# lucadellalib/ts-asr

Measured on AMD Instinct MI355X. Metric: utterance-frames/sec (conformer-t_scratch training step, T=1000, B=32/GPU), higher is better.
Workload: dtype bf16; 1 GPU; BASELINE.json configs[1]: conformer-t_scratch 12L d256 (+6L speaker encoder), mel [32,1000,80] + enrollment mel [32,500,80] + tokens [32,120], injection cat, dropout 0.1, lens 1.0; global_batch=32, grad_accumulation_factor=1, parallelism=dp1, hip_graph=True

## Files before the change

include/tsasr_hip.h:

```cpp
#ifndef TSASR_HIP_H
#define TSASR_HIP_H
#include <stddef.h>
#include <stdint.h>

#ifdef __cplusplus
extern "C" {
#endif

#define TSASR_F32 0
#define TSASR_BF16 1

#define TSASR_E_INVALID (-1)
#define TSASR_E_LAUNCH (-2)
#define TSASR_E_WORKSPACE (-3)

const char *tsasr_last_error(void);
int tsasr_version(void);
int tsasr_device_ok(void);

int tsasr_joint_fwd(const void *enc, const void *dec, const float *W, const float *bias, float *logits,
                    int B, int T, int U1, int J, int V, int ldl, int io_dtype, float slope, void *stream);

int tsasr_joint_f32_fwd(const float *enc, const float *dec, const float *W, const float *bias, float *logits, int B, int T, int U1, int J, int V,
                        int ldl, float slope, void *stream);
// ... 77 lines not shown
                          float p, unsigned long long seed, const unsigned long long *seed_dev, const int32_t *valid_lens, int Trows,
                          int io_dtype, void *stream);
int tsasr_dropout_add_bwd(const void *dout, void *dx, float *dbias, long long M, int N, float alpha, float p,
                          unsigned long long seed, const unsigned long long *seed_dev, const int32_t *valid_lens, int Trows, int io_dtype,
                          void *workspace, size_t workspace_bytes, void *stream);
int tsasr_dropout_add2_fwd(const void *x, const float *bias, const void *res, void *out, long long M, int N, float alpha, float p,
                           unsigned long long seed, float p2, unsigned long long seed2, const unsigned long long *seed_dev,
                           const int32_t *valid_lens, int Trows, int io_dtype, void *stream);
int tsasr_dropout_add2_bwd(const void *dout, void *dx, void *dres, float *dbias, long long M, int N, float alpha, float p,
                           unsigned long long seed, float p2, unsigned long long seed2, const unsigned long long *seed_dev,
                           const int32_t *valid_lens, int Trows, int io_dtype, void *workspace, size_t workspace_bytes, void *stream);


int tsasr_convmod_fwd(const void *y2, const float *b2, const float *conv_w, const float *conv_b, const float *gamma,
                      const float *beta, void *z, void *c_save, float *mean, float *rstd, int B, int T, int D, int K, int causal,
                      float eps, float slope, int io_dtype, void *stream);
size_t tsasr_convmod_bwd_workspace_bytes(int B, int T, int D, int K);
int tsasr_convmod_bwd(const void *dz, const void *y2, const float *b2, const float *conv_w, const float *gamma, const float *beta,
                      const void *c_save, const float *mean, const float *rstd, void *dy2, float *dparams, int B, int T, int D,
                      int K, int causal, float slope, int io_dtype, void *workspace, size_t workspace_bytes, void *stream);


int tsasr_conv3x3s2_fwd(const void *x, const void *Wm, const float *b1, const void *W2, const float *b2, void *y1, void *y2, int B, int T, int F,
                        int Ci, int Co, int causal, void *stream);
size_t tsasr_conv3x3s2_wgrad_workspace_bytes(int B, int T, int F, int Ci);
int tsasr_conv3x3s2_wgrad(const void *dy1, const void *dy2, const void *x, float *dWm, float *dW2, int B, int T, int F, int Ci, int Co, int causal,
                          void *workspace, size_t workspace_bytes, void *stream);
int tsasr_conv3x3s2_wgrad_filters(const void *dy1, const void *dy2, const void *x, float *dW1, float *dW2, int B, int T, int F, int Ci, int Co, int causal,
                                  void *workspace, size_t workspace_bytes, void *stream);
size_t tsasr_conv3x3s2_dgrad_plan_bytes(int B, int T, int F, int causal);
int tsasr_conv3x3s2_dgrad_plan(int B, int T, int F, int causal, void *plan_host, size_t plan_bytes);
int tsasr_conv3x3s2_dgrad(const void *dy1, const void *dy2, const void *Wm, const void *W2, void *dx, int B, int T, int F, int Ci, int Co, int causal,
                          const void *plan_dev, size_t plan_bytes, void *stream);
int tsasr_frontend_out_len(int n);
int tsasr_frontend_c1_fwd(const void *x, const float *w1, const float *b1, const float *w2, const float *b2, void *y1, void *y2,
                          int B, int T, int F, int C, int causal, int io_dtype, void *stream);
size_t tsasr_frontend_c1_bwd_workspace_bytes(int C);
int tsasr_frontend_c1_bwd(const void *x, const void *dy1, const void *dy2, float *dparams, int B, int T, int F, int C, int causal,
                          int io_dtype, void *workspace, size_t workspace_bytes, void *stream);
int tsasr_frontend_im2col(const void *x, void *A, int B, int T, int F, int C, int causal, int io_dtype, void *stream);
int tsasr_frontend_col2im(const void *dA, const void *dR, void *dx, int B, int T, int F, int C, int causal, int io_dtype, void *stream);

int tsasr_frontend_block_supported(int Fo, int C);
int tsasr_frontend_block_fwd(const void *x, const void *y1, const void *y2, const float *w1, const float *b1, const float *w2,
                             const float *b2, const float *g1, const float *be1, const float *g2, const float *be2, void *out,
                             float *stats, int B, int T, int F, int C, int causal, float slope, float eps, float p_inner,
                             unsigned long long seed_inner, float p_outer, unsigned long long seed_outer,
                             const unsigned long long *seed_dev, int io_dtype, void *stream);
size_t tsasr_frontend_block_dparams(int Fo, int C, int with_conv);
size_t tsasr_frontend_block_bwd_workspace_bytes(int Fo, int C, int with_conv);
int tsasr_frontend_block_bwd(const void *x, const void *y1, const void *y2, const void *dout, const float *w1, const float *b1,
                             const float *w2, const float *b2, const float *g1, const float *be1, const float *g2,
                             const float *stats, void *dy1, void *dy2, float *dparams, int B, int T, int F, int C, int causal,
                             float slope, float p_inner, unsigned long long seed_inner, float p_outer,
                             unsigned long long seed_outer, const unsigned long long *seed_dev, int io_dtype, void *workspace,
                             size_t workspace_bytes, void *stream);


size_t tsasr_relpos_attn_lds_bytes(void);
int tsasr_relpos_attn_fwd(const void *qkv, const void *pk, const float *bias_u, const float *bias_v, const int32_t *key_lens,
                          void *out, float *lse, int B, int T, int H, int Dh, float scale, int causal, float pdrop,
                          unsigned long long seed, const unsigned long long *seed_dev, int io_dtype, void *stream);
size_t tsasr_relpos_attn_fwd_workspace_bytes(int B, int T, int H);
int tsasr_relpos_attn_fwd_ws(const void *qkv, const void *pk, const float *bias_u, const float *bias_v, const int32_t *key_lens,
                             void *out, float *lse, int B, int T, int H, int Dh, float scale, int causal, float pdrop,
                             unsigned long long seed, const unsigned long long *seed_dev, int io_dtype, void *workspace,
// ... 274 lines not shown
```

ts-asr_amd/_capi.py:

```python
import ctypes
import os

_HERE = os.path.dirname(os.path.abspath(__file__))
LIB_PATH = os.environ.get("TSASR_HIP_LIB") or os.path.join(_HERE, "lib", "libtsasr_hip.so")

F32, BF16 = 0, 1


class TsasrHipMissing(RuntimeError):
    pass


class TsasrHipError(RuntimeError):
    pass


_lib = None

c_void_p, c_int, c_float, c_size_t = ctypes.c_void_p, ctypes.c_int, ctypes.c_float, ctypes.c_size_t
c_double = ctypes.c_double
c_ll, c_ull = ctypes.c_longlong, ctypes.c_ulonglong

_PROTOS = {
    "tsasr_last_error": (ctypes.c_char_p, []),
# ... 23 lines not shown
    "tsasr_joint_wide_loss_error_word_offset": (ctypes.c_longlong, [c_int] * 5),
    "tsasr_joint_wide_loss_fwd": (c_int, [c_void_p] * 5 + [c_int] + [c_void_p] * 3 + [c_int] * 7 + [c_float, c_void_p, c_size_t, c_void_p]),
    "tsasr_joint_wide_loss_bwd": (c_int, [c_void_p] * 5 + [c_int] + [c_void_p] * 7 + [c_int] * 7 + [c_float, c_void_p, c_size_t, c_void_p]),
    "tsasr_joint_wide_align_workspace_bytes": (c_size_t, [c_int] * 5),
    "tsasr_joint_wide_align": (c_int, [c_void_p] * 5 + [c_int] + [c_void_p] * 3 + [c_int, c_void_p] + [c_int] * 7 + [c_float, c_void_p, c_size_t, c_void_p]),
    "tsasr_layernorm_fwd":(c_int, [c_void_p] * 6 + [c_ll, c_int, c_float, c_float, c_int, c_void_p]),
    "tsasr_layernorm_bwd_workspace_bytes": (c_size_t, [c_ll, c_int]),
    "tsasr_layernorm_bwd": (c_int, [c_void_p] * 9 + [c_ll, c_int, c_float, c_int, c_void_p, c_size_t, c_void_p]),
    "tsasr_layernorm_bwd_add": (c_int, [c_void_p] * 10 + [c_ll, c_int, c_float, c_int, c_void_p, c_size_t, c_void_p]),
    "tsasr_seed_advance": (c_int, [c_void_p, c_ull, c_void_p]),
    "tsasr_bias_act_dropout_fwd": (c_int, [c_void_p] * 3 + [c_ll, c_int, c_float, c_float, c_ull, c_void_p, c_int, c_void_p]),
    "tsasr_colpart_workspace_bytes": (c_size_t, [c_ll, c_int]),
    "tsasr_bias_act_dropout_bwd": (c_int, [c_void_p] * 4 + [c_ll, c_int, c_float, c_float, c_ull, c_void_p, c_int, c_void_p, c_size_t, c_void_p]),
    "tsasr_dropout_add_fwd": (c_int, [c_void_p] * 4 + [c_ll, c_int, c_float, c_float, c_ull, c_void_p, c_void_p, c_int, c_int, c_void_p]),
    "tsasr_dropout_add_bwd": (c_int, [c_void_p] * 3 + [c_ll, c_int, c_float, c_float, c_ull, c_void_p, c_void_p, c_int, c_int, c_void_p, c_size_t, c_void_p]),
    "tsasr_dropout_add2_fwd": (c_int, [c_void_p] * 4 + [c_ll, c_int, c_float, c_float, c_ull, c_float, c_ull, c_void_p, c_void_p, c_int, c_int, c_void_p]),
    "tsasr_dropout_add2_bwd": (c_int, [c_void_p] * 4 + [c_ll, c_int, c_float, c_float, c_ull, c_float, c_ull, c_void_p, c_void_p, c_int, c_int, c_void_p, c_size_t, c_void_p]),
    "tsasr_colsum_workspace_bytes": (c_size_t, [c_ll, c_int]),
    "tsasr_colsum": (c_int, [c_void_p, c_void_p, c_ll, c_int, c_int, c_int, c_void_p, c_size_t, c_void_p]),
    "tsasr_convmod_fwd": (c_int, [c_void_p] * 10 + [c_int] * 5 + [c_float, c_float, c_int, c_void_p]),
    "tsasr_convmod_bwd_workspace_bytes": (c_size_t, [c_int] * 4),
    "tsasr_convmod_bwd": (c_int, [c_void_p] * 11 + [c_int] * 5 + [c_float, c_int, c_void_p, c_size_t, c_void_p]),
    "tsasr_frontend_out_len": (c_int, [c_int]),
    "tsasr_frontend_c1_fwd": (c_int, [c_void_p] * 7 + [c_int] * 6 + [c_void_p]),
    "tsasr_frontend_c1_bwd_workspace_bytes": (c_size_t, [c_int]),
    "tsasr_frontend_c1_bwd": (c_int, [c_void_p] * 4 + [c_int] * 6 + [c_void_p, c_size_t, c_void_p]),
    "tsasr_conv3x3s2_fwd": (c_int, [c_void_p] * 7 + [c_int] * 6 + [c_void_p]),
    "tsasr_conv3x3s2_wgrad_workspace_bytes": (c_size_t, [c_int] * 4),
    "tsasr_conv3x3s2_wgrad": (c_int, [c_void_p] * 5 + [c_int] * 6 + [c_void_p, c_size_t, c_void_p]),
    "tsasr_conv3x3s2_wgrad_filters": (c_int, [c_void_p] * 5 + [c_int] * 6 + [c_void_p, c_size_t, c_void_p]),
    "tsasr_conv3x3s2_dgrad_plan_bytes": (c_size_t, [c_int] * 4),
    "tsasr_conv3x3s2_dgrad_plan": (c_int, [c_int] * 4 + [c_void_p, c_size_t]),
    "tsasr_conv3x3s2_dgrad": (c_int, [c_void_p] * 5 + [c_int] * 6 + [c_void_p, c_size_t, c_void_p]),
    "tsasr_frontend_im2col": (c_int, [c_void_p] * 2 + [c_int] * 6 + [c_void_p]),
    "tsasr_frontend_col2im": (c_int, [c_void_p] * 3 + [c_int] * 6 + [c_void_p]),
    "tsasr_frontend_block_supported": (c_int, [c_int, c_int]),
    "tsasr_frontend_block_fwd": (c_int, [c_void_p] * 13 + [c_int] * 5 + [c_float, c_float, c_float, c_ull, c_float, c_ull, c_void_p, c_int, c_void_p]),
    "tsasr_frontend_block_dparams": (c_size_t, [c_int] * 3),
    "tsasr_frontend_block_bwd_workspace_bytes": (c_size_t, [c_int] * 3),
    "tsasr_frontend_block_bwd": (c_int, [c_void_p] * 15 + [c_int] * 5 + [c_float, c_float, c_ull, c_float, c_ull, c_void_p, c_int, c_void_p, c_size_t, c_void_p]),
    "tsasr_relpos_attn_lds_bytes": (c_size_t, []),
    "tsasr_relpos_attn_fwd": (c_int, [c_void_p] * 7 + [c_int] * 4 + [c_float, c_int, c_float, c_ull, c_void_p, c_int, c_void_p]),
    "tsasr_relpos_attn_fwd_workspace_bytes": (c_size_t, [c_int] * 3),
    "tsasr_relpos_attn_fwd_ws": (c_int, [c_void_p] * 7 + [c_int] * 4 + [c_float, c_int, c_float, c_ull, c_void_p, c_int, c_void_p, c_size_t, c_void_p]),
    "tsasr_relpos_attn_bwd_workspace_bytes": (c_size_t, [c_int] * 3),
    "tsasr_relpos_attn_bwd": (c_int, [c_void_p] * 12 + [c_int] * 4 + [c_float, c_int, c_float, c_ull, c_void_p, c_int, c_void_p, c_size_t, c_void_p]),
    "tsasr_relpos_dpk_defer": (c_int, [c_int]),
    "tsasr_relpos_dpk_pending": (c_int, []),
    "tsasr_relpos_dpk_table_bytes": (c_size_t, [c_int]),
    "tsasr_relpos_dpk_flush": (c_int, [c_void_p, c_void_p, c_size_t, c_void_p]),
    "tsasr_relpos_dpk_discard": (None, []),
    "tsasr_relpos_attn_keepbits_bytes": (c_size_t, [c_int] * 3),
    "tsasr_relpos_attn_keepbits": (None, [c_void_p]),
    "tsasr_accumulate_many": (c_int, [c_void_p, c_int, c_void_p]),
    "tsasr_clip_adamw_workspace_bytes": (c_size_t, []),
    "tsasr_clip_adamw_step": (c_int, [c_void_p] * 8 + [c_ll] + [c_float] * 5 + [c_void_p, c_size_t, c_void_p]),
    "tsasr_gemm_set_plan": (None, [c_int, c_int]),
    "tsasr_gemm_set_ring": (None, [c_int]),
    "tsasr_gemm_set_lab_floor": (None, [c_int]),
    "tsasr_gemm_bf16_workspace_bytes": (c_size_t, [c_int] * 4),
    "tsasr_gemm_f32": (c_int, [c_void_p] * 3 + [c_int] * 3 + [c_ll] * 3 + [c_int] * 3 + [c_void_p]),
    "tsasr_gemm_bf16_nt_batched": (c_int, [c_void_p] * 3 + [c_int] * 3 + [c_ll] * 4 + [c_int, c_void_p]),
    "tsasr_gemm_bf16_fused_workspace_bytes": (c_size_t, [c_int] * 2),
    "tsasr_gemm_bf16_fused": (c_int, [c_void_p] * 3 + [c_int] * 3 + [c_ll] * 3 + [c_int] * 3 + [c_void_p, c_void_p, c_ll, c_float, c_float, c_ull, c_void_p, c_void_p, c_void_p, c_void_p, c_size_t, c_void_p]),
    "tsasr_gemm_bf16_fused_mask_ok": (c_int, [c_int] * 3),
    "tsasr_gemm_bf16": (c_int, [c_void_p] * 3 + [c_int] * 3 + [c_ll] * 3 + [c_int] * 4 + [c_void_p, c_size_t, c_void_p]),
# ... 177 lines not shown
```

ts-asr_amd/csrc/gemm.hip:

```cpp
#include <stdlib.h>
#include <string.h>

#include <algorithm>
#include <utility>
#include <vector>

#include "common.h"

#define GB_K 64

typedef __attribute__((address_space(3))) bf16x4 lds_bf16x4_t;

struct EpiArgs {
    int mode;
    const float *bias;
    const bf16_t *y;
    long long ldy;
    float slope, p;
    unsigned long long seed;
    const unsigned long long *seed_dev;
    float *colpart;
    const void *const *btab;
    long long c_batch;
};

template <int BM, int BN, bool AT, bool BT>
struct GemmSmem {
    static constexpr int A_LD = AT ? (BM + 32) : (GB_K + 8);
    static constexpr int B_LD = BT ? (BN + 32) : (GB_K + 8);
    static constexpr int A_ELEMS = AT ? GB_K * A_LD : BM * A_LD;
    static constexpr int B_ELEMS = BT ? GB_K * B_LD : BN * B_LD;
    static constexpr int STAGE = A_ELEMS + B_ELEMS;
    static constexpr size_t PIPE_BYTES = (size_t)2 * STAGE * sizeof(bf16_t);
    static constexpr size_t EPI_BYTES = (size_t)BM * (BN + 4) * sizeof(float);
    static constexpr size_t BYTES = PIPE_BYTES > EPI_BYTES ? PIPE_BYTES : EPI_BYTES;
};
// ... 1045 lines not shown
        const char *as = smem + (kt % RING_STAGES) * SLOT, *bs = as + TA::BYTES;
        bf16x8 af[2][NS], bfr[NS];
#pragma unroll
        for (int s = 0; s < NS; ++s) {
#pragma unroll
            for (int i = 0; i < 2; ++i) af[i][s] = TA::frag_at(as, a_off[i][s]);
            bfr[s] = TB::frag_at(bs, b_off[s]);
        }
#pragma unroll
        for (int s = 0; s < NS; ++s)
#pragma unroll
            for (int i = 0; i < 2; ++i) acc[i] = __builtin_amdgcn_mfma_f32_32x32x16_bf16(af[i][s], bfr[s], acc[i], 0, 0, 0);
    }
    asm volatile("s_waitcnt lgkmcnt(0)" ::: "memory");
    __builtin_amdgcn_s_barrier();
    constexpr int LDT = 64 + 8;
    bf16_t *tl = reinterpret_cast<bf16_t *>(smem);
    const int r = lane & 31, hh = lane >> 5;
#pragma unroll
    for (int i = 0; i < 2; ++i)
#pragma unroll
        for (int gq = 0; gq < 16; ++gq) tl[(wm * 64 + 32 * i + (gq & 3) + 8 * (gq >> 2) + 4 * hh) * LDT + wn * 32 + r] = (bf16_t)acc[i][gq];
    __syncthreads();
    for (int e = threadIdx.x; e < 128 * 8; e += 256) {
        const int rr = e >> 3, cc = (e & 7) * 8;
        const int row = r0 + rr;
        if (row >= c.rows) continue;
        const unsigned q = (unsigned)row / (unsigned)c.nf, fi_i = (unsigned)row - q * (unsigned)c.nf, b = q / (unsigned)c.nt, ti_i = q - b * (unsigned)c.nt;
        const long long pix = ((long long)b * g.T + c.t0 + c.tstep * (int)ti_i) * g.F + c.f0 + c.fstep * (int)fi_i;
        *reinterpret_cast<uint4 *>(dx + pix * g.Ci + n0 + cc) = *reinterpret_cast<const uint4 *>(tl + rr * LDT + cc);
    }
}

struct ConvAxisClass { int i0, step, n, ostep, ns, k[4], c[4]; };
static int conv_src_index_host(int o, int k, int n, int mode) {
    if (mode == 1) { const int i = 2 * o + k - 2; return i < 0 ? -1 : i; }
    int i = 2 * o + k - 1;
    if (mode == 0) { if (i < 0) i = -i; if (i >= n) i = 2 * (n - 1) - i; return i; }
    return (i < 0 || i >= n) ? -1 : i;
}
static bool conv_dgrad_axis(int n, int No, int mode, std::vector<ConvAxisClass> &out) {
    std::vector<std::vector<std::pair<int, int>>> L(n);
    for (int o = 0; o < No; ++o)
        for (int k = 0; k < 3; ++k) {
            const int i = conv_src_index_host(o, k, n, mode);
            if (i >= 0) L[i].push_back({k, o});
        }
    const int off = mode == 1 ? 2 : 1;
    std::vector<char> regular(n);
    for (int i = 0; i < n; ++i) {
        std::vector<std::pair<int, int>> e;
        for (int k = 0; k < 3; ++k)
            if (((i - k + off) & 1) == 0) {
                const int o = (i - k + off) / 2;
                if (i - k + off >= 0 && o < No) e.push_back({k, o});
            }
        std::sort(e.begin(), e.end());
        std::sort(L[i].begin(), L[i].end());
        regular[i] = e == L[i];
    }
    for (int i = 0; i < n; ++i) {
        if (regular[i]) {
            if (i >= 2 && regular[i - 2]) continue;
            ConvAxisClass a{};
            a.i0 = i; a.step = 2; a.ostep = 1; a.n = 0;
            for (int j = i; j < n && regular[j]; j += 2) ++a.n;
// ... 207 lines not shown
        p.splits = cdiv(K, p.kchunk);
        return p;
    }
    const long long t0 = (long long)cdiv(M, 128) * cdiv(N, 128), t1 = (long long)cdiv(M, 128) * cdiv(N, 64),
                    t2 = (long long)cdiv(M, 64) * cdiv(N, 64);
    static const int thr0 = 512, thr1 = 192;
    p.tile = t0 >= thr0 ? 0 : (t1 >= thr1 ? 1 : 2);
    const long long tiles = p.tile == 0 ? t0 : (p.tile == 1 ? t1 : t2);
    p.splits = 1;
    static const int min_k = 384;
    if (out_f32 && tiles < 256 && K >= min_k) {
        static const int target = 768;
        int s = (int)((target + tiles - 1) / tiles);
        const int max_s = std::max(1, K / (min_k >= 1024 ? 256 : 128));
        if (s > max_s) s = max_s;
        if (s > 32) s = 32;
        if (s < 1) s = 1;
        p.splits = s;
    }
    p.kchunk = cdiv(cdiv(K, p.splits), GB_K) * GB_K;
    p.splits = cdiv(K, p.kchunk);
    return p;
}

template <int OUT_MODE>
static void launch_tile(int tile, int tA, int tB, const void *A, const void *B, void *C, int M, int N, int K, long long lda, long long ldb,
                        long long ldc, int splits, int kchunk, long long slab_stride, hipStream_t st, const EpiArgs &ep = EpiArgs{}) {
    if (tile == 0) launch_t<128, 128, OUT_MODE>(tA, tB, A, B, C, M, N, K, lda, ldb, ldc, splits, kchunk, slab_stride, st, ep);
    else if (tile == 1) launch_t<128, 64, OUT_MODE>(tA, tB, A, B, C, M, N, K, lda, ldb, ldc, splits, kchunk, slab_stride, st, ep);
    else launch_t<64, 64, OUT_MODE>(tA, tB, A, B, C, M, N, K, lda, ldb, ldc, splits, kchunk, slab_stride, st, ep);
}

static int tile_bm(int tile) { return tile == 2 ? 64 : 128; }

extern "C" {

void tsasr_gemm_set_ring(int on) { g_use_ring = on; }
void tsasr_gemm_set_plan(int tile, int splits) { g_force_tile = tile; g_force_splits = splits; }
void tsasr_gemm_set_lab_floor(int floor_mode) { g_lab_floor = floor_mode; }

size_t tsasr_gemm_bf16_workspace_bytes(int M, int N, int K, int out_dtype) {
    const GemmPlan p = plan(M, N, K, out_dtype == TSASR_F32);
    return p.splits > 1 ? align_up((size_t)p.splits * M * N * sizeof(float), 256) : 0;
}

int tsasr_gemm_bf16(const void *A, const void *B, void *C, int M, int N, int K, long long lda, long long ldb, long long ldc,
                    int transA, int transB, int out_dtype, int accumulate, void *workspace, size_t workspace_bytes, void *stream) {
    TSASR_CHECK_ARG(A && B && C, "tsasr_gemm_bf16: null pointer");
    TSASR_CHECK_ARG(M > 0 && N > 0 && K > 0, "tsasr_gemm_bf16: empty problem (%d,%d,%d)", M, N, K);
    TSASR_CHECK_ARG(lda % 8 == 0 && ldb % 8 == 0 && (transA ? M : K) % 8 == 0 && (transB ? N : K) % 8 == 0,
                    "tsasr_gemm_bf16: rows must be multiples of 8 bf16 (M=%d N=%d K=%d lda=%lld ldb=%lld)", M, N, K, lda, ldb);
    TSASR_CHECK_ARG(out_dtype == TSASR_BF16 || out_dtype == TSASR_F32, "tsasr_gemm_bf16: bad out_dtype %d", out_dtype);
    TSASR_CHECK_ARG(!(accumulate && out_dtype != TSASR_F32), "tsasr_gemm_bf16: accumulate needs fp32 output");
    const GemmPlan p = plan(M, N, K, out_dtype == TSASR_F32);
    hipStream_t st = (hipStream_t)stream;
    static const bool log_small = false;
    if (log_small && (long long)cdiv(M, tile_bm(p.tile)) * cdiv(N, p.tile == 0 ? 128 : 64) * p.splits <= 16)
        fprintf(stderr, "[tsasr_gemm_bf16] few tiles: M=%d N=%d K=%d tA=%d tB=%d out=%d acc=%d tile=%d splits=%d\n", M, N, K, transA, transB, out_dtype, accumulate, p.tile, p.splits);
    if (p.splits > 1) {
        TSASR_CHECK_ARG(workspace && workspace_bytes >= tsasr_gemm_bf16_workspace_bytes(M, N, K, out_dtype), "tsasr_gemm_bf16: workspace too small");
        TSASR_CHECK_ARG(N % 4 == 0 && ldc % 4 == 0, "tsasr_gemm_bf16: split-K output needs N, ldc multiples of 4");
        const long long ss = (long long)M * N;
        launch_tile<1>(p.tile, transA, transB, A, B, workspace, M, N, K, lda, ldb, N, p.splits, p.kchunk, ss, st);
        if (accumulate == 2 && ldc == N && ss < (1ll << 31) && tsasr_reduce_deferring())
            tsasr_reduce_submit((const float *)workspace, (float *)C, ss, p.splits, (int)ss, 1, st);
        else
// ... 89 lines not shown
    const int s1 = conv_wgrad_splits(P, 9 * Ci), s2 = conv_wgrad_splits(P, Ci);
    float *slab2 = (float *)((char *)workspace + align_up((size_t)s1 * 128 * 9 * Ci * sizeof(float), 256));
    const int kc1 = (int)(((P + s1 - 1) / s1 + GB_K - 1) / GB_K * GB_K), kc2 = (int)(((P + s2 - 1) / s2 + GB_K - 1) / GB_K * GB_K);
    const int z1 = (int)((P + kc1 - 1) / kc1), z2 = (int)((P + kc2 - 1) / kc2);
    conv_s2_wgrad_kernel<<<(unsigned)((9 * Ci / 64) * 2 * z1), RING_THREADS, lds, st>>>((const bf16_t *)dy1, (const bf16_t *)x, slab1, g, P, 0, 9 * Ci, kc1, z1);
    conv_s2_wgrad_kernel<<<(unsigned)((Ci / 64) * 2 * z2), RING_THREADS, lds, st>>>((const bf16_t *)dy2, (const bf16_t *)x, slab2, g, P, (causal ? 7 : 4) * Ci, Ci, kc2, z2);
    if (filter_layout) conv_filter_reduce_kernel<<<(unsigned)cdiv(128 * 9 * Ci, 256), 256, 0, st>>>(slab1, dWm, Ci, z1, (long long)128 * 9 * Ci);
    else gemm_slab_reduce_kernel<<<(unsigned)cdiv(128 * 9 * Ci / 4, 256), 256, 0, st>>>(slab1, dWm, 128, 9 * Ci, 9 * Ci, z1, (long long)128 * 9 * Ci, 0);
    gemm_slab_reduce_kernel<<<(unsigned)cdiv(128 * Ci / 4, 256), 256, 0, st>>>(slab2, dW2, 128, Ci, Ci, z2, (long long)128 * Ci, 0);
    TSASR_CHECK_LAUNCH("tsasr_conv3x3s2_wgrad");
    return 0;
}

size_t tsasr_conv3x3s2_dgrad_plan_bytes(int B, int T, int F, int causal) {
    ConvDgradPlan pl;
    if (B <= 0 || T < 2 || F < 2 || !conv_dgrad_plan(B, T, F, causal, false, pl)) return 0;
    return (size_t)(CONV_DGRAD_HDR + 32 * pl.cls.size() + 2 * (size_t)pl.slots) * sizeof(int);
}
int tsasr_conv3x3s2_dgrad_plan(int B, int T, int F, int causal, void *plan_host, size_t plan_bytes) {
    TSASR_CHECK_ARG(plan_host && B > 0 && T >= 2 && F >= 2, "tsasr_conv3x3s2_dgrad_plan: bad argument");
    ConvDgradPlan pl;
    TSASR_CHECK_ARG(conv_dgrad_plan(B, T, F, causal, true, pl), "tsasr_conv3x3s2_dgrad_plan: unsupported shape (T=%d F=%d)", T, F);
    const size_t need = (size_t)(CONV_DGRAD_HDR + 32 * pl.cls.size() + 2 * (size_t)pl.slots) * sizeof(int);
    TSASR_CHECK_ARG(plan_bytes >= need, "tsasr_conv3x3s2_dgrad_plan: buffer too small");
    int *p = (int *)plan_host;
    memset(p, 0, need);
    p[0] = (int)pl.cls.size(); p[1] = pl.slots; p[2] = CONV_DGRAD_HDR; p[3] = CONV_DGRAD_HDR + 32 * (int)pl.cls.size();
    p[4] = B; p[5] = T; p[6] = F; p[7] = causal ? 1 : 0;
    static_assert(sizeof(ConvDgradClass) == 32 * sizeof(int), "class record = 32 ints");
    memcpy(p + p[2], pl.cls.data(), pl.cls.size() * sizeof(ConvDgradClass));
    for (int w = 0; w < pl.slots; ++w) { p[p[3] + 2 * w] = pl.tile_cls[w]; p[p[3] + 2 * w + 1] = pl.tile_idx[w]; }
    return 0;
}
int tsasr_conv3x3s2_dgrad(const void *dy1, const void *dy2, const void *Wm, const void *W2, void *dx, int B, int T, int F, int Ci, int Co, int causal,
                          const void *plan_dev, size_t plan_bytes, void *stream) {
    TSASR_CHECK_ARG(dy1 && dy2 && Wm && W2 && dx && plan_dev, "tsasr_conv3x3s2_dgrad: null pointer");
    TSASR_CHECK_ARG(B > 0 && T >= 2 && F >= 2 && Co == 128 && Ci % 64 == 0 && Ci >= 64 && Ci <= 128, "tsasr_conv3x3s2_dgrad: unsupported shape (Ci=%d Co=%d)", Ci, Co);
    ConvGeom g{B, T, F, (T - 1) / 2 + 1, (F - 1) / 2 + 1, Ci, causal ? 1 : 0, causal ? 2 : 0};
    TSASR_CHECK_ARG((long long)B * T * F < (1ll << 31), "tsasr_conv3x3s2_dgrad: more than 2^31 positions");
    ConvDgradPlan pl;
    TSASR_CHECK_ARG(conv_dgrad_plan(B, T, F, causal, false, pl), "tsasr_conv3x3s2_dgrad: unsupported shape (T=%d F=%d)", T, F);
    TSASR_CHECK_ARG(plan_bytes >= (size_t)(CONV_DGRAD_HDR + 32 * pl.cls.size() + 2 * (size_t)pl.slots) * sizeof(int), "tsasr_conv3x3s2_dgrad: plan of another shape");
    constexpr int lds = RING_STAGES * (RingTile<128, false>::BYTES + RingTile<64, true>::BYTES);
    (void)hipFuncSetAttribute((const void *)conv_s2_dgrad_kernel, hipFuncAttributeMaxDynamicSharedMemorySize, lds);
    conv_s2_dgrad_kernel<<<dim3((unsigned)pl.slots, (unsigned)(Ci / 64)), RING_THREADS, lds, (hipStream_t)stream>>>(
        (const bf16_t *)dy1, (const bf16_t *)dy2, (const bf16_t *)Wm, (const bf16_t *)W2, (bf16_t *)dx, g, (const int *)plan_dev);
    TSASR_CHECK_LAUNCH("tsasr_conv3x3s2_dgrad");
    return 0;
}

size_t tsasr_gemm_bf16_fused_workspace_bytes(int M, int N) { return align_up((size_t)cdiv(M, 64) * N * sizeof(float), 256); }

int tsasr_gemm_bf16_fused_mask_ok(int M, int N, int K) { return (g_force_tile < 0 && tsasr_gemm_big_bm(M, N, K)) ? 1 : 0; }

int tsasr_gemm_bf16_fused(const void *A, const void *B, void *C, int M, int N, int K, long long lda, long long ldb, long long ldc,
                          int transA, int transB, int epi_mode, const float *bias, const void *y, long long ldy, float slope, float p,
                          unsigned long long seed, const unsigned long long *seed_dev, float *dbias, void *mask, void *workspace,
                          size_t workspace_bytes, void *stream) {
    TSASR_CHECK_ARG(A && B && C, "tsasr_gemm_bf16_fused: null pointer");
    TSASR_CHECK_ARG(M > 0 && N > 0 && K > 0 && N % 8 == 0 && ldc % 8 == 0, "tsasr_gemm_bf16_fused: N and ldc must be multiples of 8");
    TSASR_CHECK_ARG(lda % 8 == 0 && ldb % 8 == 0 && (transA ? M : K) % 8 == 0 && (transB ? N : K) % 8 == 0, "tsasr_gemm_bf16_fused: rows must be multiples of 8 bf16");
    TSASR_CHECK_ARG(epi_mode == 1 || (epi_mode == 2 && y && ldy % 8 == 0), "tsasr_gemm_bf16_fused: bad epilogue mode %d", epi_mode);
    TSASR_CHECK_ARG(!mask || (!transA && !transB && tsasr_gemm_bf16_fused_mask_ok(M, N, K)), "tsasr_gemm_bf16_fused: no mask words for this shape (ask tsasr_gemm_bf16_fused_mask_ok)");
    TSASR_CHECK_ARG(p >= 0.f && p < 1.f, "tsasr_gemm_bf16_fused: bad dropout %f", p);
    TSASR_CHECK_ARG(!(mask && slope > 1.f), "tsasr_gemm_bf16_fused: mask words need a LeakyReLU slope in [0, 1] (or none), got %f", slope);
    TSASR_CHECK_ARG(!(epi_mode == 2 && dbias) || (workspace && workspace_bytes >= tsasr_gemm_bf16_fused_workspace_bytes(M, N)), "tsasr_gemm_bf16_fused: workspace too small");
    GemmPlan pl = plan(M, N, K, 0);
    hipStream_t st = (hipStream_t)stream;
    static const bool log_small = false;
    if (log_small && (long long)cdiv(M, tile_bm(pl.tile)) * cdiv(N, pl.tile == 0 ? 128 : 64) <= 16)
        fprintf(stderr, "[tsasr_gemm_bf16_fused] few tiles: M=%d N=%d K=%d tA=%d tB=%d mode=%d tile=%d\n", M, N, K, transA, transB, epi_mode, pl.tile);
    if (!transA && !transB && g_force_tile < 0) {
        const int bm = tsasr_gemm_big_bm(M, N, K);
        float *colpart = (epi_mode == 2 && dbias) ? (float *)workspace : nullptr;
        if (bm && tsasr_gemm_big_launch(A, B, C, M, N, K, lda, ldb, ldc, epi_mode, bias, y, ldy, slope, p, seed, seed_dev, colpart, mask, st) == 0) {
            if (colpart) tsasr_reduce_submit(colpart, dbias, N, cdiv(M, bm), N, 0, st);
            TSASR_CHECK_LAUNCH("tsasr_gemm_bf16_fused");
            return 0;
        }
    }
    EpiArgs ep{};
// ... 10 lines not shown
```

ts-asr_amd/ops.py:

```python
import math
import os

import torch
import torch.nn.functional as F

from . import _capi as C
from . import prof

STATUS = {
    "joint_logits": "HIP", "rnnt_loss": "HIP", "layer_norm": "HIP", "bias_act_dropout": "HIP", "dropout_add": "HIP",
    "convmod_core": "HIP",
    "frontend_c1": "HIP", "frontend_im2col/col2im": "HIP (fp32 / other channel counts)",
    "frontend block 1 (bf16)": "HIP (frontend_block.hip: convolutions and filter gradients on MFMA)",
    "frontend block 2 (bf16, C_out = 128)": "HIP implicit GEMMs (conv_s2_fwd / conv_s2_wgrad / conv_s2_dgrad)",
    "matmul(bf16)": "HIP (gemm_bf16: fwd, dgrad, wgrad-into-arena)", "matmul(fp32 parity mode)": "HIP (gemm_f32: fp32 matrix cores; fwd, dgrad, wgrad)", "lstm(bf16 training)": "HIP persistent whole-sequence kernels (per-step kernels for other H)", "lstm(decoding / fp32 parity)": "HIP (lstm_f32: exact fp32, optional initial state)",
    "attention(fp32 parity, cross_attention injection)": "HIP (attention_f32: exact fp32)", "joint(fp32 parity)": "HIP (joint_f32)",
    "joint(32 < V <= 1024: subword vocabularies)": "HIP (joint_wide.hip: vocabulary tiles inside the kernels; bf16-rounded h / W / dlogits with bf16 OR fp32 activations - "
                                                   "an exact-fp32 wide joint is not built: compute_dtype fp32 with V > 32 runs these kernels with fp32 storage)",
    "joint + loss without logits (joint_logits: lazy, 32 < V <= 1024)": "HIP (joint_wide.hip: joint_wide_lp / joint_wide_lazy_x / joint_wide_lazy_w; V <= 32 materialises)",
    "greedy search (V <= 1024, embedding <= 1024 columns)": "HIP (search.hip: greedy_decode_kernel for V <= 63 / E <= 64, greedy_decode_wide_kernel above)",
    "beam search / LM fusion with V > 63 or an embedding past 64 columns (V, E <= 1024, beam_size <= 64)":
        "HIP (search.hip: beam_search_wide_kernel, workgroup-wide log-softmax and top-k; offline, streams, timestamps and LM fusion)",
    "injection sum / prod": "HIP (inject)", "mix_sources": "HIP (dataio.hip)", "fbank": "HIP", "sentence_norm": "HIP", "fbank_frames": "HIP", "running_norm": "HIP (features_stream.hip)",
    "fbank_frames_slots": "HIP (features.hip: the fbank frame body over per-slot sample rings)", "audio_ring_append": "HIP (features_stream.hip)",
# ... 1567 lines not shown
        C.require_gpu(x)
        xc = x.contiguous()
        B, T, Fq = xc.shape
        Co = w1.shape[0]
        f = lambda t: _f32(t).contiguous()
        y1 = torch.empty(B, _out_len(T), _out_len(Fq), Co, dtype=xc.dtype, device=xc.device)
        y2 = torch.empty_like(y1)
        with prof.region("frontend_c1_fwd"):
            C.check(C.lib().tsasr_frontend_c1_fwd(C.ptr(xc), C.ptr(f(w1)), C.ptr(f(b1)), C.ptr(f(w2)), C.ptr(f(b2)), C.ptr(y1), C.ptr(y2),
                                                  B, T, Fq, Co, int(causal), C.io_dtype(xc), C.stream_ptr()), "tsasr_frontend_c1_fwd")
        ctx.save_for_backward(xc)
        ctx.cfg = (bool(causal), Co, (w1, b1, w2, b2))
        return y1, y2

    @staticmethod
    def backward(ctx, dy1, dy2):
        (xc,) = ctx.saved_tensors
        causal, Co, prm = ctx.cfg
        B, T, Fq = xc.shape
        dpar = torch.empty(Co * 12, dtype=torch.float32, device=xc.device)
        _keep(dpar)
        ws = _ws(C.lib().tsasr_frontend_c1_bwd_workspace_bytes(Co), xc.device)
        with prof.region("frontend_c1_bwd"):
            C.check(C.lib().tsasr_frontend_c1_bwd(C.ptr(xc), C.ptr(dy1.contiguous()), C.ptr(dy2.contiguous()), C.ptr(dpar), B, T, Fq, Co,
                                                  int(causal), C.io_dtype(xc), C.ptr(ws), ws.numel(), C.stream_ptr()), "tsasr_frontend_c1_bwd")
        return (None, _pgrad(prm[0], dpar[:Co * 9]), _pgrad(prm[1], dpar[Co * 9:Co * 10]), _pgrad(prm[2], dpar[Co * 10:Co * 11]),
                _pgrad(prm[3], dpar[Co * 11:]), None)


CONV_IMPLICIT = os.environ.get("TSASR_CONV_IMPLICIT", "1") != "0"


CONV_DGRAD_IMPLICIT = os.environ.get("TSASR_CONV_DGRAD", "1") != "0"
_CONV_DGRAD_PLANS = {}


def _conv_dgrad_plan(B, T, Fq, causal, device):
    key = (B, T, Fq, bool(causal), str(device))
    if key not in _CONV_DGRAD_PLANS:
        if torch.cuda.is_current_stream_capturing():
            raise RuntimeError("front-end data-gradient plan requested for a new shape during graph capture: run one eager step of this shape first")
        n = C.lib().tsasr_conv3x3s2_dgrad_plan_bytes(B, T, Fq, int(causal))
        if n == 0:
            _CONV_DGRAD_PLANS[key] = None
        else:
            host = torch.empty(n // 4, dtype=torch.int32)
            C.check(C.lib().tsasr_conv3x3s2_dgrad_plan(B, T, Fq, int(causal), host.data_ptr(), n), "tsasr_conv3x3s2_dgrad_plan")
            _CONV_DGRAD_PLANS[key] = host.to(device)
    return _CONV_DGRAD_PLANS[key]


def _pgrad_view(dwm, Co, Ci, dtype):
    return dwm.view(Co, 3, 3, Ci).permute(0, 3, 2, 1).to(dtype)


def _pgrad_view2(dw2f, shape, dtype):
    return dw2f.view(shape).to(dtype)


class _FrontendConvFn(torch.autograd.Function):

    @staticmethod
    def forward(ctx, x, w1, b1, w2, b2, causal):
        C.require_gpu(x)
        xc = x.contiguous()
        B, T, Fq, Ci = xc.shape
# ... 26 lines not shown
        elif xc.dtype == torch.float32 and _F32_HIP_GEMM:
            y1 = (gemm_f32(A, wm, P, Co, 9 * Ci, 9 * Ci, 9 * Ci, 0, 0) + b1.float()).view(B, To, Fo, Co)
            y2 = (gemm_f32(A[:, centre * Ci:], w2m, P, Co, Ci, 9 * Ci, Ci, 0, 0) + b2.float()).view(B, To, Fo, Co)
        else:
            lib_fallback("frontend conv block 2", f"{xc.dtype}, fp32 HIP GEMM off")
            Ac = A.view(P, 9, Ci)[:, centre, :]
            y1 = F.linear(A, wm, b1.to(xc.dtype)).view(B, To, Fo, Co)
            y2 = F.linear(Ac, w2m, b2.to(xc.dtype)).view(B, To, Fo, Co)
        ctx.implicit = False
        ctx.save_for_backward(A, wm, w2m)
        ctx.cfg = (bool(causal), (B, T, Fq, Ci), Co, centre, w1.dtype, b1.dtype, w2.dtype, b2.dtype, w2.shape, hip)
        ctx.biases = (b1, b2)
        return y1, y2

    @staticmethod
    def backward(ctx, dy1, dy2):
        A, wm, w2m = ctx.saved_tensors
        causal, (B, T, Fq, Ci), Co, centre, dw1t, db1t, dw2t, db2t, w2shape, hip = ctx.cfg
        P = B * _out_len(T) * _out_len(Fq)
        g1, g2 = dy1.reshape(P, Co).contiguous(), dy2.reshape(P, Co).contiguous()
        if ctx.implicit:
            xc = A
            dwm = torch.empty(Co, Ci, 3, 3, dtype=torch.float32, device=xc.device)
            dw2f = torch.empty(Co, Ci, dtype=torch.float32, device=xc.device)
            ws = _ws(C.lib().tsasr_conv3x3s2_wgrad_workspace_bytes(B, T, Fq, Ci), xc.device)
            with prof.region("conv3x3s2_wgrad", 2.0 * P * Co * 10 * Ci):
                C.check(C.lib().tsasr_conv3x3s2_wgrad_filters(C.ptr(g1), C.ptr(g2), C.ptr(xc), C.ptr(dwm), C.ptr(dw2f), B, T, Fq, Ci, Co, int(causal),
                                                              C.ptr(ws), ws.numel(), C.stream_ptr()), "tsasr_conv3x3s2_wgrad_filters")
            db1, db2 = _pgrad(ctx.biases[0], colsum(g1)), _pgrad(ctx.biases[1], colsum(g2))
            dx = torch.empty(B, T, Fq, Ci, dtype=xc.dtype, device=xc.device)
            plan = _conv_dgrad_plan(B, T, Fq, causal, xc.device) if CONV_DGRAD_IMPLICIT else None
            if plan is not None:
                with prof.region("conv3x3s2_dgrad", 2.0 * P * Co * 10 * Ci):
                    C.check(C.lib().tsasr_conv3x3s2_dgrad(C.ptr(g1), C.ptr(g2), C.ptr(wm), C.ptr(w2m), C.ptr(dx), B, T, Fq, Ci, Co, int(causal),
                                                          C.ptr(plan), plan.numel() * 4, C.stream_ptr()), "tsasr_conv3x3s2_dgrad")
            else:
                dA = gemm_bf16(g1, wm, P, 9 * Ci, Co, Co, 9 * Ci, 0, 1)
                dR = gemm_bf16(g2, w2m, P, Ci, Co, Co, Ci, 0, 1)
                with prof.region("frontend_col2im"):
                    C.check(C.lib().tsasr_frontend_col2im(C.ptr(dA), C.ptr(dR), C.ptr(dx), B, T, Fq, Ci, int(causal), C.io_dtype(xc), C.stream_ptr()),
                            "tsasr_frontend_col2im")
            return dx, _pgrad(ctx.weights[0], dwm.to(dw1t)), db1, _pgrad(ctx.weights[1], dw2f.to(dw2t)), db2, None
        if hip:
            dwm = gemm_bf16(g1, A, Co, 9 * Ci, P, Co, 9 * Ci, 1, 1, out_dtype=torch.float32)
            dw2 = gemm_bf16(g2, A[:, centre * Ci:], Co, Ci, P, Co, 9 * Ci, 1, 1, out_dtype=torch.float32).view(w2shape).to(dw2t)
            dA = gemm_bf16(g1, wm, P, 9 * Ci, Co, Co, 9 * Ci, 0, 1)
            dR = gemm_bf16(g2, w2m, P, Ci, Co, Co, Ci, 0, 1)
        elif A.dtype == torch.float32 and _F32_HIP_GEMM:
            dwm = gemm_f32(g1, A, Co, 9 * Ci, P, Co, 9 * Ci, 1, 1)
            dw2 = gemm_f32(g2, A[:, centre * Ci:], Co, Ci, P, Co, 9 * Ci, 1, 1).view(w2shape).to(dw2t)
            dA = gemm_f32(g1, wm, P, 9 * Ci, Co, Co, 9 * Ci, 0, 1)
            dR = gemm_f32(g2, w2m, P, Ci, Co, Co, Ci, 0, 1)
        else:
            dwm = g1.t() @ A
            dw2 = (g2.t() @ A.view(P, 9, Ci)[:, centre, :]).view(w2shape).to(dw2t)
            dA = g1 @ wm
            dR = g2 @ w2m
        dw1 = dwm.view(Co, 3, 3, Ci).permute(0, 3, 2, 1).to(dw1t)
        if hip:
            db1, db2 = _pgrad(ctx.biases[0], colsum(g1)), _pgrad(ctx.biases[1], colsum(g2))
        else:
            db1, db2 = g1.sum(0, dtype=torch.float32).to(db1t), g2.sum(0, dtype=torch.float32).to(db2t)
        dx = torch.empty(B, T, Fq, Ci, dtype=A.dtype, device=A.device)
        with prof.region("frontend_col2im"):
            C.check(C.lib().tsasr_frontend_col2im(C.ptr(dA), C.ptr(dR), C.ptr(dx), B, T, Fq, Ci, int(causal), C.io_dtype(A), C.stream_ptr()),
                    "tsasr_frontend_col2im")
        return dx, dw1, db1, dw2, db2, None

# ... 766 lines not shown
```

Measured before the change: 3.270 million frames/s.

## Add persistent warp-specialized conv3x3s2 dgrad kernel with producer DMA waves

Adds a persistent version of the stride-2 conv data-gradient kernel. Four producer waves stream A/B tiles into a 3-stage LDS ring via global_load_lds, while eight consumer waves run MFMA and write dx through an LDS staging buffer. The grid is capped at the CU count and walks the plan's tile list, and BN=128 lets each tile cover both Ci halves. The host-side plan rebuild on every call is also replaced by a small cached shape table. This is meant to cut launch/tail overhead and hide load latency in the front-end backward, at the cost of a single WG per CU and more complex barrier-count coupling between the two wave groups.

```diff
diff --git a/include/tsasr_hip.h b/include/tsasr_hip.h
--- a/include/tsasr_hip.h
+++ b/include/tsasr_hip.h
@@ -133,6 +133,9 @@
 int tsasr_conv3x3s2_dgrad_plan(int B, int T, int F, int causal, void *plan_host, size_t plan_bytes);
 int tsasr_conv3x3s2_dgrad(const void *dy1, const void *dy2, const void *Wm, const void *W2, void *dx, int B, int T, int F, int Ci, int Co, int causal,
                           const void *plan_dev, size_t plan_bytes, void *stream);
+int tsasr_conv3x3s2_dgrad_impl(const void *dy1, const void *dy2, const void *Wm, const void *W2, void *dx, int B, int T, int F, int Ci, int Co,
+                               int causal, const void *plan_dev, size_t plan_bytes, int impl, void *stream);
+void tsasr_conv3x3s2_dgrad_next_wgs(int wgs);
 int tsasr_frontend_out_len(int n);
 int tsasr_frontend_c1_fwd(const void *x, const float *w1, const float *b1, const float *w2, const float *b2, void *y1, void *y2,
                           int B, int T, int F, int C, int causal, int io_dtype, void *stream);
diff --git a/ts-asr_amd/_capi.py b/ts-asr_amd/_capi.py
--- a/ts-asr_amd/_capi.py
+++ b/ts-asr_amd/_capi.py
@@ -79,6 +79,8 @@
     "tsasr_conv3x3s2_dgrad_plan_bytes": (c_size_t, [c_int] * 4),
     "tsasr_conv3x3s2_dgrad_plan": (c_int, [c_int] * 4 + [c_void_p, c_size_t]),
     "tsasr_conv3x3s2_dgrad": (c_int, [c_void_p] * 5 + [c_int] * 6 + [c_void_p, c_size_t, c_void_p]),
+    "tsasr_conv3x3s2_dgrad_impl": (c_int, [c_void_p] * 5 + [c_int] * 6 + [c_void_p, c_size_t, c_int, c_void_p]),
+    "tsasr_conv3x3s2_dgrad_next_wgs": (None, [c_int]),
     "tsasr_frontend_im2col": (c_int, [c_void_p] * 2 + [c_int] * 6 + [c_void_p]),
     "tsasr_frontend_col2im": (c_int, [c_void_p] * 3 + [c_int] * 6 + [c_void_p]),
     "tsasr_frontend_block_supported": (c_int, [c_int, c_int]),
diff --git a/ts-asr_amd/csrc/gemm.hip b/ts-asr_amd/csrc/gemm.hip
--- a/ts-asr_amd/csrc/gemm.hip
+++ b/ts-asr_amd/csrc/gemm.hip
@@ -2,6 +2,7 @@
 #include <string.h>
 
 #include <algorithm>
+#include <mutex>
 #include <utility>
 #include <vector>
 
@@ -1113,6 +1114,180 @@
     }
 }
 
+typedef const __attribute__((address_space(4))) int *conv_plan_ptr;
+typedef const __attribute__((address_space(4))) ConvDgradClass *conv_class_ptr;
+
+struct ConvDgradWalk {
+    conv_plan_ptr order;
+    int slots, G, e, cls, tile, pe, pcls, ptile;
+    __device__ __forceinline__ void request_next() {
+        pe = e + G;
+        pcls = -1; ptile = 0;
+        if (pe < slots) { pcls = order[2 * pe]; ptile = order[2 * pe + 1]; }
+    }
+    __device__ __forceinline__ void skip_padding() {
+        while (e < slots && cls < 0) {
+            e += G;
+            if (e < slots) { cls = order[2 * e]; tile = order[2 * e + 1]; }
+        }
+        request_next();
+    }
+    __device__ __forceinline__ void start(conv_plan_ptr order_, int slots_, int G_, int w) {
+        order = order_; slots = slots_; G = G_; e = w;
+        cls = -1; tile = 0;
+        if (e < slots) { cls = order[2 * e]; tile = order[2 * e + 1]; }
+        skip_padding();
+    }
+    __device__ __forceinline__ void advance() { e = pe; cls = pcls; tile = ptile; skip_padding(); }
+    __device__ __forceinline__ bool done() const { return e >= slots; }
+};
+
+__device__ __forceinline__ int conv_dgrad_tile_barriers(conv_class_ptr c) { return 2 * (c->nst * c->nsf + (c->res_st >= 0 ? 1 : 0)); }
+
+#define CONV_DGRAD_CW 8
+template <int BN>
+__global__ __launch_bounds__((CONV_DGRAD_CW + 4) * 64, 1) void conv_s2_dgrad_persistent_kernel(const bf16_t *__restrict__ dy1, const bf16_t *__restrict__ dy2,
+                                                                                   const bf16_t *__restrict__ Wm , const bf16_t *__restrict__ W2 ,
+                                                                                   bf16_t *__restrict__ dx, ConvGeom g, const int *__restrict__ plan) {
+    using TA = RingTile<128, false>;
+    using TB = RingTile<BN, true>;
+    constexpr int ST = RING_STAGES, CW = CONV_DGRAD_CW, SLOT = TA::BYTES + TB::BYTES, NS = GB_K / 16, CB = BN / 64, LPT = TA::INSTR + TB::INSTR;
+    constexpr int LDT = 32 * CB + 8, STAGE = 32 * LDT * 2;
+    static_assert(CW == 8 && LPT <= 8 && ST == 3, "ring_wait_landed covers 8 DMA instructions per k-tile, two k-tiles younger");
+    extern __shared__ __attribute__((aligned(16))) char smem[];
+    const int lane = threadIdx.x & 63, wave8 = __builtin_amdgcn_readfirstlane(threadIdx.x >> 6), wave = wave8 & 3, wm = wave8 >> 1, wn = wave8 & 1;
+    conv_plan_ptr cplan = (conv_plan_ptr)plan;
+    conv_class_ptr ctab = (conv_class_ptr)(cplan + cplan[2]);
+    const int NH = g.Ci / BN;
+    ConvDgradWalk wk;
+    wk.start(cplan + cplan[3], cplan[1], (int)gridDim.x, (int)blockIdx.x);
+    if (wave8 >= CW) {
+        const bf16_t *gb[TB::INSTR], *g2[TB::INSTR];
+        TB::src_ptrs(Wm, 9 * g.Ci, 0, g.Ci, 0, wave, lane, gb);
+        TB::src_ptrs(W2, g.Ci, 0, g.Ci, 0, wave, lane, g2);
+        int lrow[TA::INSTR], chunk[TA::INSTR];
+#pragma unroll
+        for (int i = 0; i < TA::INSTR; ++i) {
+            const int byte = (i * 4 + wave) * 1024 + lane * 16;
+            lrow[i] = byte / TA::ROW_BYTES;
+            chunk[i] = TA::swz(lrow[i], (byte % TA::ROW_BYTES) / 16) * 8;
+        }
+        conv_class_ptr c = ctab;
+        int rb[TA::INSTR], rit[TA::INSTR], rif[TA::INSTR], nki = 0, nreg = 0, kti = 0, h = 0, islot = 0;
+        auto place = [&]() {
+            c = ctab + wk.cls;
+            nki = conv_dgrad_tile_barriers(c);
+            nreg = c->nst * c->nsf;
+            const int r0 = wk.tile * 128;
+#pragma unroll
+            for (int i = 0; i < TA::INSTR; ++i) {
+                const unsigned row = (unsigned)min(r0 + lrow[i], c->rows - 1), q = row / (unsigned)c->nf;
+                rif[i] = (int)(row - q * (unsigned)c->nf);
+                rb[i] = (int)(q / (unsigned)c->nt);
+                rit[i] = (int)(q - (unsigned)rb[i] * (unsigned)c->nt);
+            }
+        };
+        auto issue_next = [&]() {
+            char *slot = smem + islot * SLOT;
+            islot = islot + 1 == ST ? 0 : islot + 1;
+            const int sl = kti >> 1, half = kti & 1;
+            const bool res = sl >= nreg;
+            const int st = res ? c->res_st : sl / c->nsf, sf = res ? c->res_sf : sl - st * c->nsf;
+            const int ct = c->ct[st], cf = c->cf[sf];
+            const bf16_t *src = (res ? dy2 : dy1) + half * GB_K;
+#pragma unroll
+            for (int i = 0; i < TA::INSTR; ++i) {
+                const int to = rit[i] * c->ost + ct, fo = rif[i] * c->osf + cf;
+                const bool ok = (unsigned)to < (unsigned)g.To && (unsigned)fo < (unsigned)g.Fo;
+                const bf16_t *p = ok ? src + ((long long)(rb[i] * g.To + to) * g.Fo + fo) * 128 + chunk[i] : g_conv_zero_line + chunk[i];
+                __builtin_amdgcn_global_load_lds((const __attribute__((address_space(1))) void *)p,
+                                                 (__attribute__((address_space(3))) void *)(slot + (i * 4 + wave) * 1024), 16, 0, 0);
+            }
+            const long long boff = res ? (long long)half * GB_K * g.Ci + h * BN : (long long)half * GB_K * 9 * g.Ci + (c->kt[st] * 3 + c->kf[sf]) * g.Ci + h * BN;
+#pragma unroll
+            for (int i = 0; i < TB::INSTR; ++i)
+                __builtin_amdgcn_global_load_lds((const __attribute__((address_space(1))) void *)((res ? g2[i] : gb[i]) + boff),
+                                                 (__attribute__((address_space(3))) void *)(slot + TA::BYTES + (i * 4 + wave) * 1024), 16, 0, 0);
+            if (++kti == nki) {
+                kti = 0;
+                if (++h == NH) {
+                    h = 0;
+                    wk.advance();
+                    if (!wk.done()) place();
+                }
+            }
+        };
+        if (!wk.done()) place();
+        int issued = 0, consumed = 0;
+        for (int t = 0; t < ST - 1; ++t)
+            if (!wk.done()) { issue_next(); ++issued; }
+        while (consumed < issued) {
+            ring_wait_landed(issued - consumed - 1, LPT);
+            __builtin_amdgcn_s_barrier();
+            ++consumed;
+            if (!wk.done()) { issue_next(); ++issued; }
+        }
+        return;
+    }
+    int a_off[NS][TA::NFO], b_off[CB][NS][TB::NFO];
+#pragma unroll
+    for (int s = 0; s < NS; ++s) {
+        TA::frag_offsets(wm * 32, s, lane, a_off[s]);
+#pragma unroll
+        for (int j = 0; j < CB; ++j) TB::frag_offsets(wn * (BN / 2) + 32 * j, s, lane, b_off[j][s]);
+    }
+    bf16_t *tl = reinterpret_cast<bf16_t *>(smem + ST * SLOT + wave8 * STAGE);
+    const int r = lane & 31, hh = lane >> 5;
+    constexpr int CPR = 4 * CB, RPI = 64 / CPR;
+    int cslot = 0;
+    while (!wk.done()) {
+        conv_class_ptr c = ctab + wk.cls;
+        const int nk = conv_dgrad_tile_barriers(c), r0 = wk.tile * 128 + wm * 32;
+        const int rows = c->rows, nf = c->nf, nt = c->nt, t0 = c->t0, tstep = c->tstep, f0 = c->f0, fstep = c->fstep;
+        for (int h = 0; h < NH; ++h) {
+            f32x16 acc[CB];
+#pragma unroll
+            for (int j = 0; j < CB; ++j) acc[j] = (f32x16){0};
+            for (int kt = 0; kt < nk; ++kt) {
+                __builtin_amdgcn_s_barrier();
+                const char *as = smem + cslot * SLOT, *bs = as + TA::BYTES;
+                cslot = cslot + 1 == ST ? 0 : cslot + 1;
+                bf16x8 af[NS], bfr[CB][NS];
+#pragma unroll
+                for (int s = 0; s < NS; ++s) {
+                    af[s] = TA::frag_at(as, a_off[s]);
+#pragma unroll
+                    for (int j = 0; j < CB; ++j) bfr[j][s] = TB::frag_at(bs, b_off[j][s]);
+                }
+                __builtin_amdgcn_sched_barrier(0);
+#pragma unroll
+                for (int s = 0; s < NS; ++s)
+#pragma unroll
+                    for (int j = 0; j < CB; ++j) acc[j] = __builtin_amdgcn_mfma_f32_32x32x16_bf16(af[s], bfr[j][s], acc[j], 0, 0, 0);
+            }
+            asm volatile("s_waitcnt lgkmcnt(0)" ::: "memory");
+            const int n0 = h * BN + wn * (BN / 2);
+#pragma unroll
+            for (int j = 0; j < CB; ++j)
+#pragma unroll
+                for (int gq = 0; gq < 16; ++gq) tl[((gq & 3) + 8 * (gq >> 2) + 4 * hh) * LDT + 32 * j + r] = (bf16_t)acc[j][gq];
+            asm volatile("" ::: "memory");
+#pragma unroll
+            for (int it = 0; it < 32 / RPI; ++it) {
+                const int rr = it * RPI + lane / CPR, cc = (lane % CPR) * 8;
+                const int row = r0 + rr;
+                if (row < rows) {
+                    const unsigned q = (unsigned)row / (unsigned)nf, fi_i = (unsigned)row - q * (unsigned)nf, b = q / (unsigned)nt, ti_i = q - b * (unsigned)nt;
+                    const long long pix = ((long long)b * g.T + t0 + tstep * (int)ti_i) * g.F + f0 + fstep * (int)fi_i;
+                    *reinterpret_cast<uint4 *>(dx + pix * g.Ci + n0 + cc) = *reinterpret_cast<const uint4 *>(tl + rr * LDT + cc);
+                }
+            }
+            asm volatile("" ::: "memory");
+        }
+        wk.advance();
+    }
+}
+
 struct ConvAxisClass { int i0, step, n, ostep, ns, k[4], c[4]; };
 static int conv_src_index_host(int o, int k, int n, int mode) {
     if (mode == 1) { const int i = 2 * o + k - 2; return i < 0 ? -1 : i; }
@@ -1386,6 +1561,38 @@
 }
 
 static int tile_bm(int tile) { return tile == 2 ? 64 : 128; }
+
+struct ConvDgradShape { int B, T, F, causal, ncls, slots; };
+static bool conv_dgrad_shape(int B, int T, int F, int causal, int &ncls, int &slots) {
+    constexpr int KEEP = 16;
+    static std::mutex mu;
+    static ConvDgradShape kept[KEEP];
+    static int used = 0, next = 0;
+    std::lock_guard<std::mutex> lock(mu);
+    for (int i = 0; i < used; ++i)
+        if (kept[i].B == B && kept[i].T == T && kept[i].F == F && kept[i].causal == causal) {
+            ncls = kept[i].ncls; slots = kept[i].slots;
+            return slots >= 0;
+        }
+    ConvDgradPlan pl;
+    const bool ok = conv_dgrad_plan(B, T, F, causal, false, pl);
+    ncls = (int)pl.cls.size(); slots = ok ? pl.slots : -1;
+    kept[next] = ConvDgradShape{B, T, F, causal, ncls, slots};
+    next = (next + 1) % KEEP;
+    used = std::min(used + 1, KEEP);
+    return ok;
+}
+
+static int g_dgrad_next_wgs = 0;
+template <int BN>
+static void conv_dgrad_persistent_launch(const void *dy1, const void *dy2, const void *Wm, const void *W2, void *dx, const ConvGeom &g, const void *plan_dev,
+                                         int G, hipStream_t st) {
+    constexpr int lds = RING_STAGES * (RingTile<128, false>::BYTES + RingTile<BN, true>::BYTES) + CONV_DGRAD_CW * 32 * (BN / 2 + 8) * 2;
+    static_assert(lds <= 160 * 1024, "ring + staging blocks fit a CU's LDS");
+    (void)hipFuncSetAttribute((const void *)conv_s2_dgrad_persistent_kernel<BN>, hipFuncAttributeMaxDynamicSharedMemorySize, lds);
+    conv_s2_dgrad_persistent_kernel<BN><<<dim3((unsigned)G), (CONV_DGRAD_CW + 4) * 64, lds, st>>>((const bf16_t *)dy1, (const bf16_t *)dy2, (const bf16_t *)Wm, (const bf16_t *)W2,
+                                                                                           (bf16_t *)dx, g, (const int *)plan_dev);
+}
 
 extern "C" {
 
@@ -1541,21 +1748,39 @@
     for (int w = 0; w < pl.slots; ++w) { p[p[3] + 2 * w] = pl.tile_cls[w]; p[p[3] + 2 * w + 1] = pl.tile_idx[w]; }
     return 0;
 }
+void tsasr_conv3x3s2_dgrad_next_wgs(int wgs) { g_dgrad_next_wgs = wgs; }
+
+int tsasr_conv3x3s2_dgrad_impl(const void *dy1, const void *dy2, const void *Wm, const void *W2, void *dx, int B, int T, int F, int Ci, int Co, int causal,
+                               const void *plan_dev, size_t plan_bytes, int impl, void *stream) {
+    const int cap = g_dgrad_next_wgs;
+    g_dgrad_next_wgs = 0;
+    TSASR_CHECK_ARG(dy1 && dy2 && Wm && W2 && dx && plan_dev, "tsasr_conv3x3s2_dgrad: null pointer");
+    TSASR_CHECK_ARG(B > 0 && T >= 2 && F >= 2 && Co == 128 && Ci % 64 == 0 && Ci >= 64 && Ci <= 128, "tsasr_conv3x3s2_dgrad: unsupported shape (Ci=%d Co=%d)", Ci, Co);
+    TSASR_CHECK_ARG(impl >= 0 && impl <= 2, "tsasr_conv3x3s2_dgrad: impl %d", impl);
+    ConvGeom g{B, T, F, (T - 1) / 2 + 1, (F - 1) / 2 + 1, Ci, causal ? 1 : 0, causal ? 2 : 0};
+    TSASR_CHECK_ARG((long long)B * T * F < (1ll << 31), "tsasr_conv3x3s2_dgrad: more than 2^31 positions");
+    int ncls = 0, slots = 0;
+    TSASR_CHECK_ARG(conv_dgrad_shape(B, T, F, causal ? 1 : 0, ncls, slots), "tsasr_conv3x3s2_dgrad: unsupported shape (T=%d F=%d)", T, F);
+    TSASR_CHECK_ARG(plan_bytes >= (size_t)(CONV_DGRAD_HDR + 32 * (size_t)ncls + 2 * (size_t)slots) * sizeof(int), "tsasr_conv3x3s2_dgrad: plan of another shape");
+    if (impl == 1 && Ci == 64) impl = 0;
+    if (impl == 0) {
+        constexpr int lds = RING_STAGES * (RingTile<128, false>::BYTES + RingTile<64, true>::BYTES);
+        (void)hipFuncSetAttribute((const void *)conv_s2_dgrad_kernel, hipFuncAttributeMaxDynamicSharedMemorySize, lds);
+        conv_s2_dgrad_kernel<<<dim3((unsigned)slots, (unsigned)(Ci / 64)), RING_THREADS, lds, (hipStream_t)stream>>>(
+            (const bf16_t *)dy1, (const bf16_t *)dy2, (const bf16_t *)Wm, (const bf16_t *)W2, (bf16_t *)dx, g, (const int *)plan_dev);
+    } else {
+        static const int cus = [] { hipDeviceProp_t pr; int d = 0; (void)hipGetDevice(&d); return hipGetDeviceProperties(&pr, d) == hipSuccess && pr.multiProcessorCount >= 8 ? pr.multiProcessorCount : 256; }();
+        int G = std::min(slots, cus / 8 * 8);
+        if (cap > 0) G = std::min(G, std::max(8, cap / 8 * 8));
+        if (impl == 1) conv_dgrad_persistent_launch<128>(dy1, dy2, Wm, W2, dx, g, plan_dev, G, (hipStream_t)stream);
+        else conv_dgrad_persistent_launch<64>(dy1, dy2, Wm, W2, dx, g, plan_dev, G, (hipStream_t)stream);
+    }
+    TSASR_CHECK_LAUNCH("tsasr_conv3x3s2_dgrad");
+    return 0;
+}
 int tsasr_conv3x3s2_dgrad(const void *dy1, const void *dy2, const void *Wm, const void *W2, void *dx, int B, int T, int F, int Ci, int Co, int causal,
                           const void *plan_dev, size_t plan_bytes, void *stream) {
-    TSASR_CHECK_ARG(dy1 && dy2 && Wm && W2 && dx && plan_dev, "tsasr_conv3x3s2_dgrad: null pointer");
-    TSASR_CHECK_ARG(B > 0 && T >= 2 && F >= 2 && Co == 128 && Ci % 64 == 0 && Ci >= 64 && Ci <= 128, "tsasr_conv3x3s2_dgrad: unsupported shape (Ci=%d Co=%d)", Ci, Co);
-    ConvGeom g{B, T, F, (T - 1) / 2 + 1, (F - 1) / 2 + 1, Ci, causal ? 1 : 0, causal ? 2 : 0};
-    TSASR_CHECK_ARG((long long)B * T * F < (1ll << 31), "tsasr_conv3x3s2_dgrad: more than 2^31 positions");
-    ConvDgradPlan pl;
-    TSASR_CHECK_ARG(conv_dgrad_plan(B, T, F, causal, false, pl), "tsasr_conv3x3s2_dgrad: unsupported shape (T=%d F=%d)", T, F);
-    TSASR_CHECK_ARG(plan_bytes >= (size_t)(CONV_DGRAD_HDR + 32 * pl.cls.size() + 2 * (size_t)pl.slots) * sizeof(int), "tsasr_conv3x3s2_dgrad: plan of another shape");
-    constexpr int lds = RING_STAGES * (RingTile<128, false>::BYTES + RingTile<64, true>::BYTES);
-    (void)hipFuncSetAttribute((const void *)conv_s2_dgrad_kernel, hipFuncAttributeMaxDynamicSharedMemorySize, lds);
-    conv_s2_dgrad_kernel<<<dim3((unsigned)pl.slots, (unsigned)(Ci / 64)), RING_THREADS, lds, (hipStream_t)stream>>>(
-        (const bf16_t *)dy1, (const bf16_t *)dy2, (const bf16_t *)Wm, (const bf16_t *)W2, (bf16_t *)dx, g, (const int *)plan_dev);
-    TSASR_CHECK_LAUNCH("tsasr_conv3x3s2_dgrad");
-    return 0;
+    return tsasr_conv3x3s2_dgrad_impl(dy1, dy2, Wm, W2, dx, B, T, F, Ci, Co, causal, plan_dev, plan_bytes, 1, stream);
 }
 
 size_t tsasr_gemm_bf16_fused_workspace_bytes(int M, int N) { return align_up((size_t)cdiv(M, 64) * N * sizeof(float), 256); }
diff --git a/ts-asr_amd/ops.py b/ts-asr_amd/ops.py
--- a/ts-asr_amd/ops.py
+++ b/ts-asr_amd/ops.py
@@ -1623,6 +1623,7 @@
 
 
 CONV_DGRAD_IMPLICIT = os.environ.get("TSASR_CONV_DGRAD", "1") != "0"
+CONV_DGRAD_PERSISTENT = int(os.environ.get("TSASR_CONV_DGRAD_PERSISTENT", "1"))
 _CONV_DGRAD_PLANS = {}
 
 
@@ -1715,8 +1716,8 @@
             plan = _conv_dgrad_plan(B, T, Fq, causal, xc.device) if CONV_DGRAD_IMPLICIT else None
             if plan is not None:
                 with prof.region("conv3x3s2_dgrad", 2.0 * P * Co * 10 * Ci):
-                    C.check(C.lib().tsasr_conv3x3s2_dgrad(C.ptr(g1), C.ptr(g2), C.ptr(wm), C.ptr(w2m), C.ptr(dx), B, T, Fq, Ci, Co, int(causal),
-                                                          C.ptr(plan), plan.numel() * 4, C.stream_ptr()), "tsasr_conv3x3s2_dgrad")
+                    C.check(C.lib().tsasr_conv3x3s2_dgrad_impl(C.ptr(g1), C.ptr(g2), C.ptr(wm), C.ptr(w2m), C.ptr(dx), B, T, Fq, Ci, Co, int(causal),
+                                                               C.ptr(plan), plan.numel() * 4, int(CONV_DGRAD_PERSISTENT), C.stream_ptr()), "tsasr_conv3x3s2_dgrad")
             else:
                 dA = gemm_bf16(g1, wm, P, 9 * Ci, Co, Co, 9 * Ci, 0, 1)
                 dR = gemm_bf16(g2, w2m, P, Ci, Co, Co, Ci, 0, 1)
```

Result: no change. 3.297 million frames/s, median of 6 (+0.8%).
